# ChainUpZero/baby-plonk-rust

Hardware: AMD Instinct MI355X
Metric: g1_msm_scalar_muls_per_s (higher is better)
Workload: dtype u32 limbs (381-bit Fp Montgomery, 255-bit Fr)

## Files before the change

baby_plonk_rust_amd/csrc/capi_ctx.hip:

```cpp
#include <stdlib.h>
#include <string.h>

#include <algorithm>
#include <chrono>
#include <condition_variable>
#include <functional>
#include <mutex>
#include <thread>
#include <vector>

#include "ctx.hpp"

#include "capi_common.hpp"

using namespace bp;

namespace bp {

int fail(bp_ctx* ctx, int code, const char* what, hipError_t e, const char* file, int line) {
  if (ctx) {
    char buf[512];
    snprintf(buf, sizeof buf, "%s%s%s (%s:%d)", what, e != hipSuccess ? ": " : "", e != hipSuccess ? hipGetErrorString(e) : "", file,
             line);
    ctx->last_error = buf;
  }
  return code;
}

static thread_local bool tl_member_worker = false;

hipError_t stream_wait(hipStream_t st) {
  static const bool block = [] { const char* v = knob("BP_WAIT_BLOCK"); return v && *v == '1'; }();
  if (!block) {
    const auto limit = tl_member_worker ? std::chrono::microseconds(50) : std::chrono::microseconds(6000);
    const auto t0 = std::chrono::steady_clock::now();
    for (uint32_t spins = 0;; spins++) {
      const hipError_t e = hipStreamQuery(st);
      if (e != hipErrorNotReady) return e;
      __builtin_ia32_pause();
      if ((spins & 15) == 15 && std::chrono::steady_clock::now() - t0 > limit) break;
    }
  }
  return hipStreamSynchronize(st);
}

int ws_get(bp_ctx* ctx, const char* name, size_t bytes, void** out) {
  DevBuf& b = ctx->ws[name];
  if (bytes == 0) bytes = 16;
  if (b.cap < bytes) {
    if (b.p) {
      BP_HIP(ctx, stream_wait(ctx->stream));
      BP_HIP(ctx, hipFree(b.p));
      b.p = nullptr;
      b.cap = 0;
    }
    size_t cap = (bytes + 255) & ~(size_t)255;
    BP_HIP(ctx, hipMalloc(&b.p, cap));
    b.cap = cap;
  }
  *out = b.p;
  return BP_OK;
}

int ev_get(bp_ctx* ctx, const char* name, size_t count, unsigned flags, hipEvent_t** out) {
  std::vector<hipEvent_t>& ev = ctx->events[name];
  while (ev.size() < count) {
    hipEvent_t e;
    BP_HIP(ctx, hipEventCreateWithFlags(&e, flags));
    ev.push_back(e);
  }
  *out = ev.data();
  return BP_OK;
}

int pinned_get(bp_ctx* ctx, size_t bytes, void** out) {
  if (ctx->pinned_cap < bytes) {
    if (ctx->pinned) BP_HIP(ctx, hipHostFree(ctx->pinned));
    ctx->pinned = nullptr;
    ctx->pinned_cap = 0;
    size_t cap = std::max<size_t>(bytes, 64 * 1024);
    BP_HIP(ctx, hipHostMalloc(&ctx->pinned, cap, hipHostMallocDefault));
    ctx->pinned_cap = cap;
  }
  *out = ctx->pinned;
  return BP_OK;
}

}

int upload_fr(bp_ctx* ctx, const char* name, const void* host, size_t n, size_t cap_elems, int fmt, fr_t** out, uint32_t* d_bad) {
  fr_t* d;
  BP_TRY(ws_get(ctx, name, std::max(cap_elems, n) * sizeof(fr_t), (void**)&d));
  if (n) BP_HIP(ctx, hipMemcpyAsync(d, host, n * sizeof(fr_t), hipMemcpyHostToDevice, ctx->stream));
  if (fmt == BP_FR_BYTES_LE) BP_TRY(fr_convert_run(ctx, d, n, 0, d_bad));
  *out = d;
  return BP_OK;
}
int download_fr(bp_ctx* ctx, fr_t* d, void* host, size_t n, int fmt, const uint32_t* d_bad) {
  if (n == 0 && !d_bad) return BP_OK;
  uint32_t bad = 0;
  if (n && fmt == BP_FR_BYTES_LE) BP_TRY(fr_convert_run(ctx, d, n, 1));
  if (n) BP_HIP(ctx, hipMemcpyAsync(host, d, n * sizeof(fr_t), hipMemcpyDeviceToHost, ctx->stream));
  if (d_bad) BP_HIP(ctx, hipMemcpyAsync(&bad, d_bad, sizeof bad, hipMemcpyDeviceToHost, ctx->stream));
  BP_HIP(ctx, stream_wait(ctx->stream));
  if (bad) return BP_FAIL(ctx, BP_ERR_BAD_SCALAR, "vector element >= q");
  return BP_OK;
}

namespace bp {
struct MemberWorker {
  std::mutex mu;
  std::condition_variable cv;
  std::function<void()> job;
  bool has_job = false, done = true, stop = false;
  std::thread th;
  MemberWorker() : th([this] { loop(); }) {}
  ~MemberWorker() {
    {
      std::lock_guard<std::mutex> lk(mu);
      stop = true;
    }
    cv.notify_all();
    th.join();
  }
  void loop() {
    tl_member_worker = true;
    std::unique_lock<std::mutex> lk(mu);
    for (;;) {
      cv.wait(lk, [&] { return has_job || stop; });
      if (stop) return;
      std::function<void()> j = std::move(job);
      has_job = false;
      lk.unlock();
      j();
// ... 220 lines not shown
```

baby_plonk_rust_amd/csrc/ctx.hpp:

```cpp
#pragma once
#include <hip/hip_runtime.h>
#include <stdint.h>
#include <stdio.h>
#include <stdlib.h>
#include <map>
#include <string>
#include <vector>

#include "../../include/bp_msm_ntt.h"
#include "g1.hpp"
#include "g1_28.hpp"
#include "msm_plan.hpp"
#include "ntt_plan.hpp"
#include "prover_host.hpp"

namespace bp {

#ifdef BP_EXPERIMENT
inline const char* knob(const char* name) { return getenv(name); }
constexpr bool EXPERIMENT_BUILD = true;
#else
inline const char* knob(const char*) { return nullptr; }
constexpr bool EXPERIMENT_BUILD = false;
#endif
// ... 136 lines not shown
  const void* gen_table_ptr = nullptr;
  void* pinned = nullptr;
  size_t pinned_cap = 0;
};

namespace bp {

int fail(bp_ctx* ctx, int code, const char* what, hipError_t e, const char* file, int line);

inline int& device_guard_depth() {
  static thread_local int depth = 0;
  return depth;
}
struct DeviceGuard {
  int prev = -1;
  explicit DeviceGuard(int device) {
    if (device_guard_depth()++ == 0) (void)hipGetLastError();
    if (hipGetDevice(&prev) != hipSuccess) prev = -1;
    if (prev != device) (void)hipSetDevice(device);
  }
  ~DeviceGuard() {
    int cur = -1;
    if (prev >= 0 && hipGetDevice(&cur) == hipSuccess && cur != prev) (void)hipSetDevice(prev);
    device_guard_depth()--;
  }
  DeviceGuard(const DeviceGuard&) = delete;
  DeviceGuard& operator=(const DeviceGuard&) = delete;
};
inline bool is_group(const bp_ctx* ctx) { return ctx->members.size() > 1; }
inline int lift(bp_ctx* ctx, const bp_ctx* member, int rc) {
  if (rc != BP_OK && member != ctx) ctx->last_error = member->last_error;
  return rc;
}
inline bool peer_path(const bp_ctx* m, int other_device) {
  if (m->device != other_device) return true;
  if (m->leader && m->leader->rehearsal) return true;
  const char* v = knob("BP_FORCE_PEER_COPIES");
  return v && *v && *v != '0';
}

#define BP_HIP(ctx, call)                                                              \
  do {                                                                                 \
    hipError_t e__ = (call);                                                           \
    if (e__ != hipSuccess) return ::bp::fail(ctx, BP_ERR_HIP, #call, e__, __FILE__, __LINE__); \
  } while (0)
#define BP_FAIL(ctx, code, text) ::bp::fail(ctx, code, text, hipSuccess, __FILE__, __LINE__)
#define BP_TRY(expr)              \
  do {                            \
    int rc__ = (expr);            \
    if (rc__ != BP_OK) return rc__; \
  } while (0)

hipError_t stream_wait(hipStream_t st);
struct StreamDrain {
  hipStream_t st;
  ~StreamDrain() { (void)stream_wait(st); }
};

int ws_get(bp_ctx* ctx, const char* name, size_t bytes, void** out);
int ev_get(bp_ctx* ctx, const char* name, size_t count, unsigned flags, hipEvent_t** out);
int pinned_get(bp_ctx* ctx, size_t bytes, void** out);

struct MsmPending {
  bool empty = true, blob = false;
  bool tables = false;
  uint32_t c = 0, Wr = 0, n_planes = 0;
  uint32_t quads = 1;
  uint32_t J = 1;
  uint64_t adds = 0;
  const void* h_windows = nullptr;
};
int msm_launch(bp_ctx* ctx, const g1_affine28* d_points28, size_t n, const fr_t* d_scalars, int fmt, uint32_t table_c, size_t table_stride,
               int slot, void* d_blob, MsmPending* out);
int msm_launch_many(bp_ctx* ctx, const g1_affine28* d_points28, uint32_t J, const fr_t* const* d_scalars_each, const size_t* n_each, int fmt,
                    uint32_t table_c, size_t table_stride, int slot, void* d_blob, MsmPending* out);
int msm_blobs_combine(const uint8_t* blobs, size_t n_blobs, g1_proj* out);
int msm_blobs_sum_device_run(bp_ctx* ctx, const void* d_blobs, size_t n_blobs, void* d_out, bool wait = true);
int msm_blob_poisoned(const uint8_t* blobs, size_t n_blobs, uint32_t* rank);
int msm_blob_poison_run(bp_ctx* ctx, void* d_blob, int err, uint32_t rank);
int msm_finish(bp_ctx* ctx, const MsmPending& pend, g1_proj* host_out);
struct MsmFlight {
  bp_ctx* on = nullptr;
  MsmPending pend;
  bool launched = false;
  int rc = BP_OK;
  g1_proj out[MSM_MAX_BATCH];
};
inline int msm_flight_launched(MsmFlight& f, bp_ctx* on, int launch_rc) {
  f.on = on;
  f.rc = launch_rc;
  f.launched = launch_rc == BP_OK;
  return launch_rc;
}
int msm_finish_all(bp_ctx* ctx, MsmFlight* f, size_t count, int rc);
int msm_run(bp_ctx* ctx, const g1_affine28* d_points28, size_t n, const fr_t* d_scalars, int fmt, uint32_t table_c, size_t table_stride,
            g1_proj* host_out);
int msm_init_device(bp_ctx* ctx);
int commit_many(bp_ctx* ctx, uint64_t srs_handle, const fr_t* const* d_coeffs, const size_t* n, int k, g1_proj* out);
int srs_tables_run(bp_ctx* ctx, const g1_affine* d_points, const g1_affine28* d_points28, size_t n, uint32_t c, g1_affine28** d_table,
                   uint32_t* windows);
MsmKnobs msm_knobs();
int srs_to28_run(bp_ctx* ctx, const g1_affine* d_in, size_t n, g1_affine28** d_out);
int srs_to28_into(bp_ctx* ctx, const g1_affine* d_in, size_t n, g1_affine28* d_out);
int ntt_init_tables(bp_ctx* ctx);
int ntt_run(bp_ctx* ctx, fr_t* d_data, uint32_t log_n, int inverse, size_t batch, size_t stride);
NttKnobs ntt_knobs();
int ntt_tmp_buffer(bp_ctx* ctx, uint32_t log_n, fr_t** out);
int ntt_run_part(bp_ctx* ctx, const NttHostPlan& plan, fr_t* d_data, int inverse, size_t batch, size_t stride, int phase, uint32_t part, uint32_t parts);
int fr_convert_run(bp_ctx* ctx, fr_t* d, size_t n, int dir, uint32_t* d_bad = nullptr);
int fr_flag_noncanonical_run(bp_ctx* ctx, const fr_t* d, size_t n, uint32_t* d_bad, size_t row = 0, size_t stride = 0);
int fr_bad_word(bp_ctx* ctx, int fmt, uint32_t** d_bad);
int fr_binary_run(bp_ctx* ctx, const fr_t* a, size_t na, const fr_t* b, size_t nb, fr_t* out, size_t n, int op);
int fr_scalar_run(bp_ctx* ctx, const fr_t* a, const fr_t& s, fr_t* out, size_t n, int op);
int poly_eval_run(bp_ctx* ctx, const fr_t* d_coeffs, size_t n, const fr_t& x, fr_t* host_out, const uint32_t* d_bad = nullptr);
int poly_eval_many_run(bp_ctx* ctx, int k, const fr_t* const* d_coeffs, const size_t* n, const fr_t* x, fr_t* host_out);
int poly_div_run(bp_ctx* ctx, fr_t* d_a, size_t na, const fr_t* d_b, size_t nb, const fr_t& b0, const fr_t& b_lead, bool binomial,
                 fr_t* d_q, size_t nq);
int fr_nonzero_stats_run(bp_ctx* ctx, const fr_t* d_a, size_t n, size_t lo, size_t hi, size_t* eff_len, size_t* nonzero_in_range);
int fr_compact_nonzero_run(bp_ctx* ctx, fr_t* d_q, size_t* n);
int fr_squeeze_zeros_run(bp_ctx* ctx, fr_t* d_q, size_t* n);
int fr_scale_powers_run(bp_ctx* ctx, const fr_t* d_a, size_t n, const fr_t& w, fr_t* d_out);
int fr_synthetic_run(bp_ctx* ctx, fr_t* d_out, size_t n, uint64_t seed);
int fr_scan_mul_run(bp_ctx* ctx, const fr_t* d_in, size_t n, int reverse, int inclusive, fr_t* d_out, fr_t* d_total);
// ... 45 lines not shown
```

baby_plonk_rust_amd/csrc/g1_28.hpp:

```cpp
#pragma once
#include "fp28.hpp"
#include "g1.hpp"

namespace bp {

template <class To, uint64_t A, uint32_t VA>
BP_HD To widen28(const F28<A, VA>& a) {
  static_assert(A <= To::limb_bound && VA <= To::value_bound, "cannot narrow bounds");
  To r;
#pragma unroll
  for (int i = 0; i < N28; i++) r.l[i] = a.l[i];
  return r;
}

using C28 = F28<MASK28 + 8, 6>;
using PtY28 = F28<MASK28 + 8, 2>;

struct alignas(128) g1_affine28 {
  F28n x, y;
};
struct g1_proj28 {
  C28 x, y, z;
};
constexpr int PROJ28_WORDS = 44;
// ... 33 lines not shown
#pragma unroll
  for (int i = 0; i < N28; i++) zero.l[i] = 0;
  auto ny = norm28(sub28<2, 29>(zero, y));
  PtY28 a = widen28<PtY28>(ny), b = widen28<PtY28>(y), r;
#pragma unroll
  for (int i = 0; i < N28; i++) r.l[i] = neg ? a.l[i] : b.l[i];
  return r;
}

BP_HD void g1_add_mixed28(g1_proj28& acc, const F28n& x2, const PtY28& y2) {
  const C28 &X1 = acc.x, &Y1 = acc.y, &Z1 = acc.z;
  auto t0 = mul28(X1, x2);
  auto t1 = mul28(Y1, y2);
  auto t3 = mul28(add28(x2, y2), add28(X1, Y1));
  auto t3s = norm28(sub28<8, 30>(t3, add28(t0, t1)));
  auto t4 = add28(mul28(y2, Z1), Y1);
  auto y3a = norm28(add28(mul28(x2, Z1), X1));
  auto t0x3 = mulk28<3>(t0);
  auto t2 = norm28(mulk28<12>(Z1));
  auto z3 = add28(t1, t2);
  auto t1s = sub28<80, 29>(t1, t2);
  auto y3 = norm28(mulk28<12>(y3a));
  auto x3 = mul28_2(t3s, t1s, t4, neg28<128, 29>(y3));
  auto yo = mul28_2(t1s, z3, y3, t0x3);
  auto zo = mul28_2(z3, t4, t0x3, t3s);
  acc.x = widen28<C28>(x3);
  acc.y = widen28<C28>(yo);
  acc.z = widen28<C28>(zo);
}

BP_HD void g1_add28(g1_proj28& r, const g1_proj28& a, const g1_proj28& b) {
  auto t0 = mul28(a.x, b.x);
  auto t1 = mul28(a.y, b.y);
  auto t2 = mul28(a.z, b.z);
  auto t3 = norm28(sub28<8, 30>(mul28(add28(a.x, a.y), add28(b.x, b.y)), add28(t0, t1)));
  auto t4 = norm28(sub28<8, 30>(mul28(add28(a.y, a.z), add28(b.y, b.z)), add28(t1, t2)));
  auto y3a = norm28(sub28<8, 30>(mul28(add28(a.x, a.z), add28(b.x, b.z)), add28(t0, t2)));
  auto t0x3 = mulk28<3>(t0);
  auto t2b = norm28(mulk28<12>(t2));
  auto z3 = add28(t1, t2b);
  auto t1s = sub28<32, 29>(t1, t2b);
  auto y3 = norm28(mulk28<12>(y3a));
  auto x3 = mul28_2(t3, t1s, t4, neg28<128, 29>(y3));
  auto yo = mul28_2(t1s, z3, y3, t0x3);
  auto zo = mul28_2(z3, t4, t0x3, t3);
  r.x = widen28<C28>(x3);
  r.y = widen28<C28>(yo);
  r.z = widen28<C28>(zo);
}

using CoopProd = F28<MASK28, 2>;
using CoopSum = decltype(add28(C28(), C28()));

template <class U, class A, class B, class C>
BP_HD U select3_28(uint32_t which, const A& a, const B& b, const C& c) {
  const U ua = widen28<U>(a), ub = widen28<U>(b), uc = widen28<U>(c);
  U r;
#pragma unroll
  for (int i = 0; i < N28; i++) r.l[i] = which == 0 ? ua.l[i] : (which == 1 ? ub.l[i] : uc.l[i]);
  return r;
}
template <class A, class B, class C>
struct Union28 {
  static constexpr uint64_t lb = A::limb_bound > B::limb_bound ? (A::limb_bound > C::limb_bound ? A::limb_bound : C::limb_bound)
                                                               : (B::limb_bound > C::limb_bound ? B::limb_bound : C::limb_bound);
  static constexpr uint32_t vb = A::value_bound > B::value_bound ? (A::value_bound > C::value_bound ? A::value_bound : C::value_bound)
                                                                 : (B::value_bound > C::value_bound ? B::value_bound : C::value_bound);
  using type = F28<lb, vb>;
};

BP_HD CoopProd g1_add28_coop_a(uint32_t role, const g1_proj28& a, const g1_proj28& b) {
  const bool ux = role == 0 || role == 3 || role == 5, uy = role == 1 || role == 3 || role == 4, uz = role == 2 || role == 4 || role == 5;
  CoopSum u, v;
#pragma unroll
  for (int i = 0; i < N28; i++) {
    u.l[i] = (ux ? a.x.l[i] : 0u) + (uy ? a.y.l[i] : 0u) + (uz ? a.z.l[i] : 0u);
    v.l[i] = (ux ? b.x.l[i] : 0u) + (uy ? b.y.l[i] : 0u) + (uz ? b.z.l[i] : 0u);
  }
  return widen28<CoopProd>(mul28(u, v));
}
BP_HD C28 g1_add28_coop_b(uint32_t role, const CoopProd p[6]) {
  const CoopProd &t0 = p[0], &t1 = p[1], &t2 = p[2];
  auto t3 = norm28(sub28<8, 30>(p[3], add28(t0, t1)));
  auto t4 = norm28(sub28<8, 30>(p[4], add28(t1, t2)));
  auto y3a = norm28(sub28<8, 30>(p[5], add28(t0, t2)));
  auto t0x3 = norm28(mulk28<3>(t0));
  auto t2b = norm28(mulk28<12>(t2));
  auto z3 = norm28(add28(t1, t2b));
  auto t1s = norm28(sub28<32, 29>(t1, t2b));
  auto y3 = norm28(mulk28<12>(y3a));
  auto ny3 = norm28(neg28<128, 29>(y3));
  using P = typename Union28<decltype(t3), decltype(z3), decltype(t0x3)>::type;
  using Q = typename Union28<decltype(t1s), decltype(t1s), decltype(t3)>::type;
  using R = typename Union28<decltype(t4), decltype(t0x3), decltype(t4)>::type;
  using S = typename Union28<decltype(ny3), decltype(y3), decltype(z3)>::type;
  const uint32_t w = role < 3 ? role : 2;
  return widen28<C28>(mul28_2(select3_28<P>(w, t3, z3, t0x3), select3_28<Q>(w, t1s, t1s, t3), select3_28<R>(w, t4, t0x3, t4),
                              select3_28<S>(w, ny3, y3, z3)));
}

BP_HD void g1_double28(g1_proj28& r, const g1_proj28& p) {
  auto t0 = mul28(p.y, p.y);
  auto z8 = mulk28<8>(t0);
  auto t1 = mul28(p.y, p.z);
  auto t2 = norm28(mulk28<12>(mul28(p.z, p.z)));
  auto x3 = mul28(t2, z8);
  auto y3 = add28(t0, t2);
  auto zo = mul28(t1, z8);
  auto t0s = sub28<80, 30>(t0, mulk28<3>(t2));
  auto yo = add28(x3, mul28(t0s, y3));
  auto xo = mulk28<2>(mul28(t0s, mul28(p.x, p.y)));
  r.x = widen28<C28>(norm28(xo));
// ... 46 lines not shown
```

baby_plonk_rust_amd/csrc/msm.hip:

```cpp
#include <math.h>
#include <stdlib.h>
#include <string.h>

#include <vector>

#include "ctx.hpp"
#include "msm_kernels.hpp"

namespace bp {

static_assert(sizeof(proj28_slot) == MSM_SLOT_BYTES, "msm_plan.hpp sizes the workspaces by this");

MsmKnobs msm_knobs() { return msm_knobs_read(knob_u32); }

int srs_to28_run(bp_ctx* ctx, const g1_affine* d_in, size_t n, g1_affine28** d_out) {
  g1_affine28* d = nullptr;
  BP_HIP(ctx, hipMalloc((void**)&d, (n ? n : 1) * sizeof(g1_affine28)));
  if (n) hipLaunchKernelGGL(srs_to28, dim3((unsigned)((n + 255) / 256)), dim3(256), 0, ctx->stream, d_in, n, d);
  BP_HIP(ctx, hipGetLastError());
  *d_out = d;
  return BP_OK;
}

int srs_to28_into(bp_ctx* ctx, const g1_affine* d_in, size_t n, g1_affine28* d_out) {
// ... 92 lines not shown
  out->blob = d_blob != nullptr;
  const MsmHostPlan hp = msm_plan(J, n_each, table_c, table_stride, d_blob != nullptr, msm_knobs());
  if (hp.err == BP_ERR_INVALID_ARG) return BP_FAIL(ctx, hp.err, hp.what);
  out->J = J;
  if (hp.empty) {
    if (d_blob) {
      MsmBlobHeader hdr;
      memset(&hdr, 0, sizeof hdr);
      hdr.magic = MSM_BLOB_MAGIC;
      hipLaunchKernelGGL(msm_write_blob, dim3(1), dim3(64), 0, ctx->stream, (const proj28_slot*)nullptr, hdr, (uint8_t*)d_blob);
      BP_HIP(ctx, hipGetLastError());
    }
    return BP_OK;
  }
  if (slot < 0 || slot >= MSM_SLOTS) return BP_FAIL(ctx, BP_ERR_INVALID_ARG, "MSM result slot");
  if (hp.err) return BP_FAIL(ctx, hp.err, hp.what);
  const MsmPlan& plan = hp.dev;
  MsmScalars scalars_all;
  for (uint32_t j = 0; j < MSM_MAX_BATCH; j++) scalars_all.p[j] = j < J ? d_scalars_each[j] : nullptr;
  SortBufs b = {};
  uint32_t* long_list;
  proj28_slot *long_scratch, *bucket_sum, *partial, *roots = nullptr, *window_sum, *tmp[2] = {nullptr, nullptr};
  const struct { const char* name; size_t bytes; void** p; } buffers[] = {
      {"msm.ctl", hp.ws.ctl, (void**)&b.ctl},
      {"msm.counts", hp.ws.counts, (void**)&b.counts},
      {"msm.offsets", hp.ws.offsets, (void**)&b.offsets},
      {"msm.cursors", hp.ws.cursors, (void**)&b.cursors},
      {"msm.long_list", hp.ws.long_list, (void**)&long_list},
      {"msm.long_scratch", hp.ws.long_scratch, (void**)&long_scratch},
      {"msm.tile_sums", hp.ws.tile_sums, (void**)&b.tile_sums},
      {"msm.sorted", hp.ws.sorted, (void**)&b.sorted},
      {"msm.bucket_sum", hp.ws.bucket_sum, (void**)&bucket_sum},
      {"msm.partial", hp.ws.partial, (void**)&partial},
      {"msm.roots", hp.ws.roots, (void**)&roots},
      {"msm.window_sum", hp.ws.window_sum, (void**)&window_sum},
      {"msm.rkeys0", hp.ws.rkeys0, (void**)&b.keys[0]},
      {"msm.rvals0", hp.ws.rvals0, (void**)&b.vals[0]},
      {"msm.rkeys1", hp.ws.rkeys1, (void**)&b.keys[1]},
      {"msm.rvals1", hp.ws.rvals1, (void**)&b.vals[1]},
      {"msm.run_off", hp.ws.run_off, (void**)&b.run_off},
      {"msm.run_cnt", hp.ws.run_cnt, (void**)&b.run_cnt},
      {"msm.run_cur", hp.ws.run_cur, (void**)&b.run_cur},
      {"msm.run_long", hp.ws.run_long, (void**)&b.run_long},
      {"msm.planes_tmp0", hp.ws.planes_tmp0, (void**)&tmp[0]},
      {"msm.planes_tmp1", hp.ws.planes_tmp1, (void**)&tmp[1]},
  };
  for (const auto& w : buffers)
    if (w.bytes) BP_TRY(ws_get(ctx, w.name, w.bytes, w.p));
  constexpr size_t slot_bytes = (size_t)MSM_MAX_WINDOWS * sizeof(proj28_slot) + 16;
  uint8_t* h_base;
  BP_TRY(pinned_get(ctx, MSM_SLOTS * slot_bytes, (void**)&h_base));
  proj28_slot* h_windows = reinterpret_cast<proj28_slot*>(h_base + (size_t)slot * slot_bytes);
  const uint32_t total = plan.total, n_planes = hp.n_planes;
  uint32_t *offsets = b.offsets, *long_count = b.ctl, *status = b.ctl + 1, *long_ticket = b.ctl + 8 + PART_MAX;
  hipStream_t st = ctx->stream;
  BP_HIP(ctx, hipEventRecord(ctx->ev[0], st));
  BP_HIP(ctx, hipMemsetAsync(b.ctl, 0, (size_t)hp.ctl_zeroed * 4, st));
  if (hp.sort == 2) {
    level1_launch(st, hp, scalars_all, fmt, b, b.run_off, b.keys[0], b.vals[0]);
    (hp.packed ? final_runs_launch<true> : final_runs_launch<false>)(st, hp, b, b.keys[0], b.vals[0], b.run_off);
  } else {
    uint32_t* const run_off[2] = {b.run_off + 4,
                                  b.run_off + 8 + hp.n_final};
    level1_launch(st, hp, scalars_all, fmt, b, run_off[0], b.keys[1], b.vals[1]);
    uint32_t side = 1;
    if (hp.lv[1]) {
      const dim3 grid(hp.gx2, 1u << hp.lv[0]);
      BP_HIP(ctx, hipMemsetAsync(b.run_cnt, 0, (size_t)hp.n_sub * 4, st));
      hipLaunchKernelGGL(msm_radix_count, grid, dim3(1024), 0, st, b.keys[side], run_off[0], hp.shift2, hp.lv[1], b.run_cnt);
      hipLaunchKernelGGL(scan_tile_sums, dim3(hp.scan_tiles), dim3(256), 0, st, b.run_cnt, hp.n_sub, b.tile_sums);
      hipLaunchKernelGGL(scan_block_sums, dim3(1), dim3(256), 0, st, b.tile_sums, hp.scan_tiles, run_off[1] + hp.n_sub);
      hipLaunchKernelGGL(scan_apply, dim3(hp.scan_tiles), dim3(256), 0, st, b.run_cnt, hp.n_sub, b.tile_sums, run_off[1], b.run_cur);
      hipLaunchKernelGGL(msm_radix_scatter, grid, dim3(1024), RADIX_SLICE * 9, st, b.keys[side], b.vals[side], run_off[0], hp.shift2, hp.lv[1], b.run_cur,
                         b.keys[side ^ 1], b.vals[side ^ 1]);
      side ^= 1;
    }
    final_runs_launch<false>(st, hp, b, b.keys[side], b.vals[side], run_off[hp.lv[1] ? 1 : 0]);
  }
  BP_HIP(ctx, hipEventRecord(ctx->ev[1], st));
  hipLaunchKernelGGL(msm_accumulate<2>, dim3(hp.acc_grid), dim3(256), 0, st, d_points28, b.sorted, offsets, plan, bucket_sum, partial);
  BP_HIP(ctx, hipEventRecord(ctx->ev[2], st));
  if (hp.by_edges)
    hipLaunchKernelGGL(msm_fixup_edges, dim3(hp.fixup_grid), dim3(256), 0, st, offsets, plan, bucket_sum, partial, long_count, long_list, hp.long_cap);
  else if (table_c)
    hipLaunchKernelGGL(msm_fixup<2>, dim3(hp.fixup_grid), dim3(256), 0, st, offsets, plan, bucket_sum, partial, long_count, long_list, hp.long_cap);
  else
    hipLaunchKernelGGL(msm_fixup<1>, dim3(hp.fixup_grid), dim3(256), 0, st, offsets, plan, bucket_sum, partial, long_count, long_list, hp.long_cap);
  hipLaunchKernelGGL(msm_fixup_long, dim3(512), dim3(256), 256 * sizeof(proj28_slot), st, offsets, plan, bucket_sum, partial, long_count, long_list, hp.long_cap,
                     long_scratch, long_ticket);
  uint32_t* const status_out = reinterpret_cast<uint32_t*>(window_sum + n_planes);
  const proj28_slot* in = bucket_sum;
  for (uint32_t i = 0; i < hp.n_steps; i++) {
    const MsmTreeStep& s = hp.step[i];
    const bool last = s.out == MSM_OUT_FINAL;
    proj28_slot* out_nodes = last ? (table_c ? window_sum : roots) : tmp[s.out];
    const dim3 grid(s.gx, s.gy);
    if (s.kind == MSM_STEP_LEVEL01) {
      hipLaunchKernelGGL(msm_planes_level01, grid, dim3(256), 0, st, offsets, in, s.nodes, out_nodes);
    } else if (s.kind == MSM_STEP_LEVEL) {
      hipLaunchKernelGGL(msm_planes_level, grid, dim3(256), 0, st, offsets, in, s.k, s.nodes, out_nodes);
    } else {
      uint32_t* so = last && table_c ? status_out : (uint32_t*)nullptr;
      if (s.k == 0) hipLaunchKernelGGL(msm_planes_step<true>, grid, dim3(256), s.lds, st, offsets, in, s.k, s.m, out_nodes, status, offsets + total, so);
      else hipLaunchKernelGGL(msm_planes_step<false>, grid, dim3(256), s.lds, st, offsets, in, s.k, s.m, out_nodes, status, offsets + total, so);
    }
    in = out_nodes;
  }
  if (!table_c)
    hipLaunchKernelGGL(msm_planes_window_quads, dim3(plan.W), dim3(64), 0, st, roots, plan.c, hp.quads, window_sum, status, offsets + total, status_out);
  BP_HIP(ctx, hipGetLastError());
  if (d_blob) {
    MsmBlobHeader hdr;
    memset(&hdr, 0, sizeof hdr);
    hdr.magic = MSM_BLOB_MAGIC;
    hdr.c = plan.c;
    hdr.Wr = table_c ? 1 : hp.Wr;
    hdr.n_planes = n_planes;
    hdr.tables = table_c != 0;
    hdr.quads = table_c ? 0u : hp.quads;
    hipLaunchKernelGGL(msm_write_blob, dim3(1), dim3(256), 0, st, window_sum, hdr, (uint8_t*)d_blob);
    BP_HIP(ctx, hipGetLastError());
  } else {
    BP_HIP(ctx, hipMemcpyAsync(h_windows, window_sum, (size_t)n_planes * sizeof(proj28_slot) + 8, hipMemcpyDeviceToHost, st));
  }
  BP_HIP(ctx, hipEventRecord(ctx->ev[3], st));
  out->empty = false;
  out->tables = table_c != 0;
  out->c = plan.c;
  out->Wr = table_c ? 1 : hp.Wr;
  out->n_planes = n_planes;
  out->quads = hp.quads;
  out->adds = hp.entries;
  out->h_windows = h_windows;
  msm_plan_path(hp, ctx->msm_path);
  return BP_OK;
}

static void host_quad_horner(g1_proj& out, const g1_proj* quads, uint32_t W, uint32_t c, uint32_t nq) {
  g1_proj acc = g1_identity();
  uint32_t prev = 0;
  bool first = true;
  for (uint32_t w = W; w-- > 0;)
    for (uint32_t j = nq; j-- > 0;) {
      const uint32_t pos = c * w + 4 * j;
      if (first) {
        acc = quads[(size_t)w * nq + j];
        first = false;
      } else {
        for (uint32_t d = pos; d < prev; d++) g1_double(acc, acc);
        g1_add(acc, acc, quads[(size_t)w * nq + j]);
      }
      prev = pos;
    }
  out = acc;
}

static void host_plane_horner(g1_proj& out, const g1_proj* planes, uint32_t W, uint32_t c) {
  g1_proj acc = g1_identity();
  for (uint32_t w = W; w-- > 0;) {
    const g1_proj* p = planes + (size_t)w * c;
    for (uint32_t j = c; j-- > 0;) {
      g1_double(acc, acc);
      if (j + 1 < c) g1_add(acc, acc, p[1 + j]);
    }
    g1_add(acc, acc, p[0]);
  }
  out = acc;
}

int msm_finish(bp_ctx* ctx, const MsmPending& pend, g1_proj* host_out) {
  ctx->msm_async_pending = false;
  if (pend.empty) {
    for (uint32_t j = 0; host_out && j < pend.J; j++) host_out[j] = g1_identity();
    ctx->msm_accumulate_ms = ctx->msm_total_ms = 0;
    ctx->msm_adds = 0;
    if (pend.blob) BP_HIP(ctx, stream_wait(ctx->stream));
    return BP_OK;
  }
  BP_HIP(ctx, stream_wait(ctx->stream));
  BP_HIP(ctx, hipEventElapsedTime(&ctx->msm_accumulate_ms, ctx->ev[1], ctx->ev[2]));
  BP_HIP(ctx, hipEventElapsedTime(&ctx->msm_total_ms, ctx->ev[0], ctx->ev[3]));
  ctx->msm_c = pend.c;
  ctx->msm_tables = pend.tables;
  ctx->msm_adds = pend.adds;
  if (pend.blob) {
    if (host_out) *host_out = g1_identity();
    return BP_OK;
  }
  const proj28_slot* h_windows = static_cast<const proj28_slot*>(pend.h_windows);
  const uint32_t n_planes = pend.n_planes;
  const uint32_t* tail = reinterpret_cast<const uint32_t*>(h_windows + n_planes);
  if (tail[0]) return BP_FAIL(ctx, BP_ERR_BAD_SCALAR, "scalar >= q in a canonical-bytes input");
  ctx->msm_adds = tail[1];
  std::vector<g1_proj> windows(n_planes);
  for (uint32_t w = 0; w < n_planes; w++) windows[w] = slot_to_proj(&h_windows[w]);
  if (pend.tables) {
    for (uint32_t j = 0; j < pend.J; j++)
      host_plane_horner(host_out[j], windows.data() + (size_t)j * pend.c, pend.Wr, pend.c);
  } else {
    host_quad_horner(*host_out, windows.data(), pend.Wr, pend.c, pend.quads);
  }
  return BP_OK;
}

int msm_blobs_combine(const uint8_t* blobs, size_t n_blobs, g1_proj* out) {
  g1_proj total = g1_identity();
  std::vector<bool> done(n_blobs, false);
  for (size_t i = 0; i < n_blobs; i++) {
    MsmBlobHeader h;
    memcpy(&h, blobs + i * BP_MSM_BLOB_BYTES, sizeof h);
    if (h.magic != MSM_BLOB_MAGIC || h.n_planes > (uint32_t)MSM_MAX_WINDOWS) return BP_ERR_INVALID_ARG;
    if (h.err != 0) return h.err < 0 && h.err >= BP_ERR_COMM ? h.err : BP_ERR_INVALID_ARG;
    if (h.tables > 1) return BP_ERR_INVALID_ARG;
    if (h.n_planes != 0) {
      const bool width_ok = h.c >= 2 && h.c <= (uint32_t)MSM_MAX_TABLE_C;
      const uint32_t per = h.tables ? h.c : (h.quads ? h.quads : 1u);
      if (!width_ok || h.Wr < 1 || per > 8 * 4 || h.n_planes != h.Wr * per) return BP_ERR_INVALID_ARG;
    }
    if (h.status) return BP_ERR_BAD_SCALAR;
  }
  for (size_t i = 0; i < n_blobs; i++) {
    if (done[i]) continue;
    MsmBlobHeader h;
    memcpy(&h, blobs + i * BP_MSM_BLOB_BYTES, sizeof h);
    done[i] = true;
    if (h.n_planes == 0) continue;
    std::vector<g1_proj> sum(h.n_planes);
    const proj28_slot* slots = reinterpret_cast<const proj28_slot*>(blobs + i * BP_MSM_BLOB_BYTES + sizeof(MsmBlobHeader));
    for (uint32_t w = 0; w < h.n_planes; w++) sum[w] = slot_to_proj(&slots[w]);
    for (size_t k = i + 1; k < n_blobs; k++) {
      MsmBlobHeader g;
      memcpy(&g, blobs + k * BP_MSM_BLOB_BYTES, sizeof g);
      if (done[k] || g.c != h.c || g.Wr != h.Wr || g.n_planes != h.n_planes || g.tables != h.tables || g.quads != h.quads) continue;
      done[k] = true;
      const proj28_slot* sk = reinterpret_cast<const proj28_slot*>(blobs + k * BP_MSM_BLOB_BYTES + sizeof(MsmBlobHeader));
      for (uint32_t w = 0; w < h.n_planes; w++) g1_add(sum[w], sum[w], slot_to_proj(&sk[w]));
    }
    g1_proj part;
    if (h.tables) host_plane_horner(part, sum.data(), h.Wr, h.c);
    else host_quad_horner(part, sum.data(), h.Wr, h.c, h.quads ? h.quads : 1u);
    g1_add(total, total, part);
  }
  *out = total;
  return BP_OK;
}

int msm_blob_poisoned(const uint8_t* blobs, size_t n_blobs, uint32_t* rank) {
  for (size_t i = 0; i < n_blobs; i++) {
    MsmBlobHeader h;
    memcpy(&h, blobs + i * BP_MSM_BLOB_BYTES, sizeof h);
    if (h.magic == MSM_BLOB_MAGIC && h.err != 0) {
      if (rank) *rank = h.err_rank;
      return h.err < 0 && h.err >= BP_ERR_COMM ? h.err : BP_ERR_INVALID_ARG;
    }
  }
// ... 31 lines not shown
```

baby_plonk_rust_amd/csrc/msm_kernels.hpp:

```cpp
#pragma once
#include "g1.hpp"
#include "g1_28.hpp"
#include "msm_digits.hpp"
#include "msm_plan.hpp"

namespace bp {

struct MsmScalars { const fr_t* p[MSM_MAX_BATCH]; };

__device__ __forceinline__ uint32_t digit_bucket(int32_t d) { return (uint32_t)(d < 0 ? -d : d) - 1u; }

extern __shared__ uint32_t msm_lds_hist[];

constexpr uint32_t SCAN_PER_LANE = 16;

__device__ __forceinline__ uint32_t block_exclusive_scan_256(uint32_t v, uint32_t* lds, uint32_t& block_total) {
  const uint32_t lane = threadIdx.x & 63, wave = threadIdx.x >> 6;
  uint32_t incl = v;
#pragma unroll
  for (int d = 1; d < 64; d <<= 1) {
    uint32_t n = __shfl_up(incl, d, 64);
    if (lane >= (uint32_t)d) incl += n;
  }
  if (lane == 63) lds[wave] = incl;
// ... 468 lines not shown

__device__ __forceinline__ g1_affine load_affine(const g1_affine* __restrict__ p) {
  g1_affine r;
  const uint4* q = reinterpret_cast<const uint4*>(p);
  uint4 v[6];
#pragma unroll
  for (int j = 0; j < 6; j++) v[j] = q[j];
#pragma unroll
  for (int j = 0; j < 3; j++) {
    r.x.l[4 * j] = v[j].x; r.x.l[4 * j + 1] = v[j].y; r.x.l[4 * j + 2] = v[j].z; r.x.l[4 * j + 3] = v[j].w;
    r.y.l[4 * j] = v[j + 3].x; r.y.l[4 * j + 1] = v[j + 3].y; r.y.l[4 * j + 2] = v[j + 3].z; r.y.l[4 * j + 3] = v[j + 3].w;
  }
  return r;
}
__device__ __forceinline__ g1_affine28 load_affine28(const g1_affine28* __restrict__ p) {
  g1_affine28 r;
  const uint4* q = reinterpret_cast<const uint4*>(p);
  uint4 v[7];
#pragma unroll
  for (int j = 0; j < 7; j++) v[j] = q[j];
  uint32_t w[28];
#pragma unroll
  for (int j = 0; j < 7; j++) { w[4 * j] = v[j].x; w[4 * j + 1] = v[j].y; w[4 * j + 2] = v[j].z; w[4 * j + 3] = v[j].w; }
#pragma unroll
  for (int j = 0; j < N28; j++) { r.x.l[j] = w[j]; r.y.l[j] = w[N28 + j]; }
  return r;
}
struct proj28_slot { uint4 q[11]; };
__device__ __forceinline__ void store_proj28(proj28_slot* __restrict__ dst, const g1_proj28& p) {
  uint32_t w[PROJ28_WORDS];
#pragma unroll
  for (int j = 0; j < N28; j++) { w[j] = p.x.l[j]; w[N28 + j] = p.y.l[j]; w[2 * N28 + j] = p.z.l[j]; }
  w[42] = 0; w[43] = 0;
#pragma unroll
  for (int j = 0; j < 11; j++) dst->q[j] = make_uint4(w[4 * j], w[4 * j + 1], w[4 * j + 2], w[4 * j + 3]);
}
__device__ __forceinline__ g1_proj28 load_proj28(const proj28_slot* __restrict__ src) {
  uint32_t w[PROJ28_WORDS];
#pragma unroll
  for (int j = 0; j < 11; j++) { uint4 v = src->q[j]; w[4 * j] = v.x; w[4 * j + 1] = v.y; w[4 * j + 2] = v.z; w[4 * j + 3] = v.w; }
  g1_proj28 p;
#pragma unroll
  for (int j = 0; j < N28; j++) { p.x.l[j] = w[j]; p.y.l[j] = w[N28 + j]; p.z.l[j] = w[2 * N28 + j]; }
  return p;
}
__device__ __forceinline__ bool is_blank28(const g1_proj28& p) {
  uint32_t z = 0;
#pragma unroll
  for (int j = 0; j < N28; j++) z |= p.z.l[j];
  return z == 0;
}

constexpr uint32_t COOP = 8;
__device__ __forceinline__ g1_proj28 g1_add28_coop(const g1_proj28& a, const g1_proj28& b) {
  const uint32_t role = threadIdx.x & (COOP - 1);
  const CoopProd mine = g1_add28_coop_a(role, a, b);
  CoopProd p[6];
#pragma unroll
  for (int r = 0; r < 6; r++) {
#pragma unroll
    for (int j = 0; j < N28; j++) p[r].l[j] = (uint32_t)__shfl((int)mine.l[j], r, COOP);
  }
  const C28 coord = g1_add28_coop_b(role, p);
  g1_proj28 out;
#pragma unroll
  for (int j = 0; j < N28; j++) {
    out.x.l[j] = (uint32_t)__shfl((int)coord.l[j], 0, COOP);
    out.y.l[j] = (uint32_t)__shfl((int)coord.l[j], 1, COOP);
    out.z.l[j] = (uint32_t)__shfl((int)coord.l[j], 2, COOP);
  }
  return out;
}

__global__ void __launch_bounds__(256) srs_to28(const g1_affine* __restrict__ in, size_t n, g1_affine28* __restrict__ out) {
  size_t i = (size_t)blockIdx.x * blockDim.x + threadIdx.x;
  if (i >= n) return;
  g1_affine28 r = g1_affine_to_28(load_affine(&in[i]));
  uint4* q = reinterpret_cast<uint4*>(&out[i]);
  uint32_t w[28];
#pragma unroll
  for (int j = 0; j < N28; j++) { w[j] = r.x.l[j]; w[N28 + j] = r.y.l[j]; }
#pragma unroll
  for (int j = 0; j < 7; j++) q[j] = make_uint4(w[4 * j], w[4 * j + 1], w[4 * j + 2], w[4 * j + 3]);
}

constexpr int TABLE_GROUP = 16;
__device__ __forceinline__ M28 one_m28() {
  M28 r;
#pragma unroll
  for (int j = 0; j < N28; j++) r.l[j] = One28::limb(j);
  return r;
}
template <bool RADIX>
__global__ void __launch_bounds__(256) srs_window_tables(const g1_affine28* __restrict__ in28, size_t n, uint32_t c, uint32_t W, uint32_t radix,
                                                         g1_affine28* __restrict__ table) {
  size_t i = (size_t)blockIdx.x * blockDim.x + threadIdx.x;
  if (i >= n) return;
  const g1_affine28 a = load_affine28(&in28[i]);
  uint32_t nz = 0;
#pragma unroll
  for (int j = 0; j < N28; j++) nz |= a.x.l[j] | a.y.l[j];
  const bool inf = nz == 0;
  g1_proj28 p = g1_identity28();
  if (!inf) {
    p.x = widen28<C28>(a.x);
    p.y = widen28<C28>(a.y);
    p.z = widen28<C28>(one_m28());
  }
  g1_proj28 row[TABLE_GROUP];
  M28 prefix[TABLE_GROUP];
  const M28 one = one_m28();
  for (uint32_t w0 = 1; w0 < W; w0 += TABLE_GROUP) {
    const uint32_t cnt = W - w0 < (uint32_t)TABLE_GROUP ? W - w0 : (uint32_t)TABLE_GROUP;
    for (uint32_t j = 0; j < cnt; j++) {
      if (RADIX) g1_mul_small28(p, p, radix, 32 - __clz(radix));
      else
// ... 248 lines not shown
    }
    g1_proj28 tot = block_tree_sum28(acc, per < blockDim.x ? per : blockDim.x);
    if (!split) {
      if (threadIdx.x == 0) store_proj28(&bucket_sum[g], tot);
      __syncthreads();
      continue;
    }
    if (threadIdx.x == 0) {
      store_proj28(&scratch[(size_t)k * FIXUP_LONG_SLICES + y], tot);
      __builtin_amdgcn_fence(__ATOMIC_RELEASE, "agent");
      asm volatile("s_waitcnt vmcnt(0)" ::: "memory");
      const uint32_t t = atomicAdd(&ticket[k], 1u);
      if (t == FIXUP_LONG_SLICES - 1) {
        ticket[k] = 0;
        __builtin_amdgcn_fence(__ATOMIC_ACQUIRE, "agent");
        asm volatile("s_waitcnt vmcnt(0)" ::: "memory");
      }
      arrived = t;
    }
    __syncthreads();
    if (arrived == FIXUP_LONG_SLICES - 1) {
      g1_proj28 v = g1_identity28();
      if (threadIdx.x < FIXUP_LONG_SLICES) v = load_proj28(&scratch[(size_t)k * FIXUP_LONG_SLICES + threadIdx.x]);
      g1_proj28 sum = block_tree_sum28(v, FIXUP_LONG_SLICES);
      if (threadIdx.x == 0) store_proj28(&bucket_sum[g], sum);
    }
    __syncthreads();
  }
}

__device__ __forceinline__ g1_proj28 block_tree_sum28(g1_proj28 v, uint32_t live) {
  proj28_slot* tree = reinterpret_cast<proj28_slot*>(msm_lds_tree);
  store_proj28(&tree[threadIdx.x], v);
  __syncthreads();
  uint32_t stride = 1;
  while (stride < live) stride <<= 1;
  const uint32_t group = threadIdx.x / COOP, n_groups = blockDim.x / COOP;
  for (stride >>= 1; stride > 0; stride >>= 1) {
    for (uint32_t i = group; i < stride; i += n_groups) {
      if (i + stride < live) {
        g1_proj28 a = load_proj28(&tree[i]), b = load_proj28(&tree[i + stride]);
        a = g1_add28_coop(a, b);
        if ((threadIdx.x & (COOP - 1)) == 0) store_proj28(&tree[i], a);
      }
    }
    __syncthreads();
  }
  return load_proj28(&tree[0]);
}


__device__ __forceinline__ proj28_slot* planes_tree(proj28_slot* cur, proj28_slot* nxt, uint32_t levels, bool planes) {
  const uint32_t group = threadIdx.x / COOP, n_groups = blockDim.x / COOP;
  const bool lead = (threadIdx.x & (COOP - 1)) == 0;
  for (uint32_t k = 0; k < levels; k++) {
    const uint32_t merges = 1u << (levels - k - 1);
    const uint32_t in_per = planes ? k + 1 : 1, out_per = planes ? k + 2 : 1, adds = merges * in_per;
    for (uint32_t item = group; item < adds; item += n_groups) {
      const uint32_t m = item / in_per, v = item - m * in_per;
      const proj28_slot* L = cur + (size_t)(2 * m) * in_per;
      g1_proj28 a = load_proj28(&L[v]), b = load_proj28(&L[in_per + v]);
      if (!(is_blank28(a) && is_blank28(b))) a = g1_add28_coop(a, b);
      if (lead) store_proj28(&nxt[(size_t)m * out_per + v], a);
    }
    if (planes)
      for (uint32_t m = threadIdx.x; m < merges; m += blockDim.x) nxt[(size_t)m * out_per + k + 1] = cur[(size_t)(2 * m + 1) * in_per];
    __syncthreads();
    proj28_slot* t = cur; cur = nxt; nxt = t;
  }
  return cur;
}

__global__ void __launch_bounds__(256, 2)
msm_planes_level(const uint32_t* __restrict__ offsets, const proj28_slot* __restrict__ in, uint32_t k, uint32_t n_out,
                 proj28_slot* __restrict__ out) {
  const uint64_t item = (uint64_t)blockIdx.x * blockDim.x + threadIdx.x;
  const uint32_t per = k + 1, node = (uint32_t)(item / per), v = (uint32_t)(item - (uint64_t)node * per);
  if (node >= n_out) return;
  const proj28_slot* L = in + (size_t)(2 * (size_t)node) * per;
  g1_proj28 a = load_proj28(&L[v]), b = load_proj28(&L[per + v]);
  proj28_slot* o = out + (size_t)node * (per + 1);
  if (v == 0) store_proj28(&o[per], b);
  if (!(is_blank28(a) && is_blank28(b))) g1_add28(a, a, b);
  store_proj28(&o[v], a);
}

__global__ void __launch_bounds__(256, 2)
msm_planes_level01(const uint32_t* __restrict__ offsets, const proj28_slot* __restrict__ in, uint32_t n_out, proj28_slot* __restrict__ out) {
  const uint32_t node = blockIdx.x * blockDim.x + threadIdx.x;
  if (node >= n_out) return;
  const size_t g = 4 * (size_t)node;
  const uint32_t o0 = offsets[g], o1 = offsets[g + 1], o2 = offsets[g + 2], o3 = offsets[g + 3], o4 = offsets[g + 4];
  proj28_slot* o = out + (size_t)node * 3;
  if (o4 == o0) {
    const g1_proj28 blank = g1_identity28();
    store_proj28(&o[0], blank);
    store_proj28(&o[1], blank);
    store_proj28(&o[2], blank);
    return;
  }
  {
    g1_proj28 s1 = o2 != o1 ? load_proj28(&in[g + 1]) : g1_identity28();
    {
      g1_proj28 a01 = o1 != o0 ? load_proj28(&in[g]) : g1_identity28();
      g1_add28(a01, a01, s1);
      store_proj28(&o[0], a01);
    }
    const g1_proj28 s3 = o4 != o3 ? load_proj28(&in[g + 3]) : g1_identity28();
    g1_add28(s1, s1, s3);
    store_proj28(&o[1], s1);
  }
  g1_proj28 a23 = o3 != o2 ? load_proj28(&in[g + 2]) : g1_identity28();
  {
    const g1_proj28 s3 = o4 != o3 ? load_proj28(&in[g + 3]) : g1_identity28();
    g1_add28(a23, a23, s3);
  }
  store_proj28(&o[2], a23);
  asm volatile("s_waitcnt vmcnt(0)" ::: "memory");
  g1_proj28 a01 = load_proj28(&o[0]);
  g1_add28(a01, a01, a23);
  store_proj28(&o[0], a01);
}

template <bool LEAF>
__global__ void __launch_bounds__(256, 2)
msm_planes_step(const uint32_t* __restrict__ offsets, const proj28_slot* __restrict__ in, uint32_t k, uint32_t m,
                proj28_slot* __restrict__ out, const uint32_t* __restrict__ status_in, const uint32_t* __restrict__ entries_in,
                uint32_t* __restrict__ status_out) {
  proj28_slot* buf = reinterpret_cast<proj28_slot*>(msm_lds_tree);
  const uint32_t w = blockIdx.x, v = blockIdx.y, nin = 1u << m, c = k + m + 1;
  if (status_out && v == 0 && w == 0 && threadIdx.x == 0) { status_out[0] = *status_in; status_out[1] = *entries_in; }
  if (threadIdx.x < nin) {
    const size_t node = ((size_t)w << m) + threadIdx.x;
    if (LEAF) {
      if (offsets[node + 1] != offsets[node]) buf[threadIdx.x] = in[node];
      else store_proj28(&buf[threadIdx.x], g1_identity28());
    } else {
      buf[threadIdx.x] = in[node * (k + 1) + v];
    }
  }
  __syncthreads();
  const proj28_slot* root = planes_tree(buf, buf + nin, m, v == 0);
  if (v == 0) {
    if (threadIdx.x == 0) out[(size_t)w * c] = root[0];
    else if (threadIdx.x <= m) out[(size_t)w * c + k + threadIdx.x] = root[threadIdx.x];
  } else if (threadIdx.x == 0) {
    out[(size_t)w * c + v] = root[0];
  }
}

__global__ void __launch_bounds__(64) msm_planes_window_quads(const proj28_slot* __restrict__ roots, uint32_t c, uint32_t nq, proj28_slot* __restrict__ window_sum,
                                                              const uint32_t* __restrict__ status_in, const uint32_t* __restrict__ entries_in,
                                                              uint32_t* __restrict__ status_out) {
  __shared__ proj28_slot part[4];
  const uint32_t w = blockIdx.x, grp = threadIdx.x / COOP, j = grp >> 1, h = grp & 1;
  const bool lead = (threadIdx.x & (COOP - 1)) == 0;
  if (w == 0 && threadIdx.x == 0) { status_out[0] = *status_in; status_out[1] = *entries_in; }
  const proj28_slot* r = roots + (size_t)w * c;
  const uint32_t np = c - 1, p0 = 4 * j + 2 * h, p1 = p0 + 1;
  auto pick = [](bool c, const g1_proj28& a, const g1_proj28& b) {
    g1_proj28 o;
#pragma unroll
    for (int i = 0; i < N28; i++) {
      o.x.l[i] = c ? a.x.l[i] : b.x.l[i];
      o.y.l[i] = c ? a.y.l[i] : b.y.l[i];
      o.z.l[i] = c ? a.z.l[i] : b.z.l[i];
    }
    return o;
  };
  const g1_proj28 blank = g1_identity28();
  const bool have1 = j < nq && p1 < np, have0 = j < nq && p0 < np;
  g1_proj28 t = pick(have1, load_proj28(&r[have1 ? 1 + p1 : 0]), blank);
  t = g1_add28_coop(t, t);
  t = g1_add28_coop(t, pick(have0, load_proj28(&r[have0 ? 1 + p0 : 0]), blank));
  t = g1_add28_coop(t, pick(h != 0, t, pick(j == 0, load_proj28(&r[0]), blank)));
  t = g1_add28_coop(t, pick(h != 0, t, blank));
  if (h && lead && j < 4) store_proj28(&part[j], t);
  __syncthreads();
  if (h) return;
  t = g1_add28_coop(t, load_proj28(&part[j]));
  if (lead && j < nq) store_proj28(&window_sum[(size_t)w * nq + j], t);
}

}
```

Baseline: 400.4 million.

## Write MSM window sums directly to mapped host memory and signal via flag

When the last tree step is a plain step kernel on the table path, its outputs go straight into coherent, mapped pinned host memory. A last-block ticket then sets a host-visible flag, so the host can start the Horner epilogue while the stream is still draining, with no D2H memcpy. The planes tree now lets three cooperating lanes each store one output coordinate instead of only the lead lane storing all of it, and select3 uses bitmask picks instead of branches. The risks are slower device writes into host-coherent memory, the pinned buffer now being mapped and coherent, and the ordering correctness of the fence and ticket.

```diff
diff --git a/baby_plonk_rust_amd/csrc/capi_ctx.hip b/baby_plonk_rust_amd/csrc/capi_ctx.hip
--- a/baby_plonk_rust_amd/csrc/capi_ctx.hip
+++ b/baby_plonk_rust_amd/csrc/capi_ctx.hip
@@ -44,6 +44,18 @@
   return hipStreamSynchronize(st);
 }
 
+bool flag_wait(const volatile uint32_t* flag) {
+  static const bool block = [] { const char* v = knob("BP_WAIT_BLOCK"); return v && *v == '1'; }();
+  if (block) return false;
+  const auto limit = tl_member_worker ? std::chrono::microseconds(50) : std::chrono::microseconds(6000);
+  const auto t0 = std::chrono::steady_clock::now();
+  for (uint32_t spins = 0;; spins++) {
+    if (__atomic_load_n(flag, __ATOMIC_ACQUIRE)) return true;
+    __builtin_ia32_pause();
+    if ((spins & 63) == 63 && std::chrono::steady_clock::now() - t0 > limit) return false;
+  }
+}
+
 int ws_get(bp_ctx* ctx, const char* name, size_t bytes, void** out) {
   DevBuf& b = ctx->ws[name];
   if (bytes == 0) bytes = 16;
@@ -79,7 +91,7 @@
     ctx->pinned = nullptr;
     ctx->pinned_cap = 0;
     size_t cap = std::max<size_t>(bytes, 64 * 1024);
-    BP_HIP(ctx, hipHostMalloc(&ctx->pinned, cap, hipHostMallocDefault));
+    BP_HIP(ctx, hipHostMalloc(&ctx->pinned, cap, hipHostMallocMapped | hipHostMallocCoherent));
     ctx->pinned_cap = cap;
   }
   *out = ctx->pinned;
diff --git a/baby_plonk_rust_amd/csrc/ctx.hpp b/baby_plonk_rust_amd/csrc/ctx.hpp
--- a/baby_plonk_rust_amd/csrc/ctx.hpp
+++ b/baby_plonk_rust_amd/csrc/ctx.hpp
@@ -212,6 +212,7 @@
   } while (0)
 
 hipError_t stream_wait(hipStream_t st);
+bool flag_wait(const volatile uint32_t* flag);
 struct StreamDrain {
   hipStream_t st;
   ~StreamDrain() { (void)stream_wait(st); }
@@ -229,6 +230,7 @@
   uint32_t J = 1;
   uint64_t adds = 0;
   const void* h_windows = nullptr;
+  const uint32_t* h_flag = nullptr;
 };
 int msm_launch(bp_ctx* ctx, const g1_affine28* d_points28, size_t n, const fr_t* d_scalars, int fmt, uint32_t table_c, size_t table_stride,
                int slot, void* d_blob, MsmPending* out);
diff --git a/baby_plonk_rust_amd/csrc/g1_28.hpp b/baby_plonk_rust_amd/csrc/g1_28.hpp
--- a/baby_plonk_rust_amd/csrc/g1_28.hpp
+++ b/baby_plonk_rust_amd/csrc/g1_28.hpp
@@ -109,12 +109,14 @@
 using CoopProd = F28<MASK28, 2>;
 using CoopSum = decltype(add28(C28(), C28()));
 
+BP_HD uint32_t pick28(uint32_t mask, uint32_t a, uint32_t b) { return (a & mask) | (b & ~mask); }
 template <class U, class A, class B, class C>
 BP_HD U select3_28(uint32_t which, const A& a, const B& b, const C& c) {
   const U ua = widen28<U>(a), ub = widen28<U>(b), uc = widen28<U>(c);
+  const uint32_t m0 = 0u - (uint32_t)(which == 0), m1 = 0u - (uint32_t)(which == 1);
   U r;
 #pragma unroll
-  for (int i = 0; i < N28; i++) r.l[i] = which == 0 ? ua.l[i] : (which == 1 ? ub.l[i] : uc.l[i]);
+  for (int i = 0; i < N28; i++) r.l[i] = pick28(m0, ua.l[i], pick28(m1, ub.l[i], uc.l[i]));
   return r;
 }
 template <class A, class B, class C>
diff --git a/baby_plonk_rust_amd/csrc/msm.hip b/baby_plonk_rust_amd/csrc/msm.hip
--- a/baby_plonk_rust_amd/csrc/msm.hip
+++ b/baby_plonk_rust_amd/csrc/msm.hip
@@ -168,6 +168,13 @@
   BP_TRY(pinned_get(ctx, MSM_SLOTS * slot_bytes, (void**)&h_base));
   proj28_slot* h_windows = reinterpret_cast<proj28_slot*>(h_base + (size_t)slot * slot_bytes);
   const uint32_t total = plan.total, n_planes = hp.n_planes;
+  const bool direct = table_c && !d_blob && hp.n_steps && hp.step[hp.n_steps - 1].kind == MSM_STEP_STEP;
+  proj28_slot* d_slot = nullptr;
+  volatile uint32_t* h_flag = reinterpret_cast<uint32_t*>(h_windows + n_planes) + 2;
+  if (direct) {
+    BP_HIP(ctx, hipHostGetDevicePointer((void**)&d_slot, h_windows, 0));
+    *h_flag = 0;
+  }
   uint32_t *offsets = b.offsets, *long_count = b.ctl, *status = b.ctl + 1, *long_ticket = b.ctl + 8 + PART_MAX;
   hipStream_t st = ctx->stream;
   BP_HIP(ctx, hipEventRecord(ctx->ev[0], st));
@@ -209,16 +216,18 @@
   for (uint32_t i = 0; i < hp.n_steps; i++) {
     const MsmTreeStep& s = hp.step[i];
     const bool last = s.out == MSM_OUT_FINAL;
-    proj28_slot* out_nodes = last ? (table_c ? window_sum : roots) : tmp[s.out];
+    proj28_slot* out_nodes = last ? (table_c ? (direct ? d_slot : window_sum) : roots) : tmp[s.out];
     const dim3 grid(s.gx, s.gy);
     if (s.kind == MSM_STEP_LEVEL01) {
       hipLaunchKernelGGL(msm_planes_level01, grid, dim3(256), 0, st, offsets, in, s.nodes, out_nodes);
     } else if (s.kind == MSM_STEP_LEVEL) {
       hipLaunchKernelGGL(msm_planes_level, grid, dim3(256), 0, st, offsets, in, s.k, s.nodes, out_nodes);
     } else {
-      uint32_t* so = last && table_c ? status_out : (uint32_t*)nullptr;
-      if (s.k == 0) hipLaunchKernelGGL(msm_planes_step<true>, grid, dim3(256), s.lds, st, offsets, in, s.k, s.m, out_nodes, status, offsets + total, so);
-      else hipLaunchKernelGGL(msm_planes_step<false>, grid, dim3(256), s.lds, st, offsets, in, s.k, s.m, out_nodes, status, offsets + total, so);
+      const bool hand_over = last && direct;
+      uint32_t* so = last && table_c ? (hand_over ? reinterpret_cast<uint32_t*>(d_slot + n_planes) : status_out) : (uint32_t*)nullptr;
+      uint32_t *ticket = hand_over ? b.ctl + 3 : (uint32_t*)nullptr, *flag = hand_over ? so + 2 : (uint32_t*)nullptr;
+      if (s.k == 0) hipLaunchKernelGGL(msm_planes_step<true>, grid, dim3(256), s.lds, st, offsets, in, s.k, s.m, out_nodes, status, offsets + total, so, ticket, flag);
+      else hipLaunchKernelGGL(msm_planes_step<false>, grid, dim3(256), s.lds, st, offsets, in, s.k, s.m, out_nodes, status, offsets + total, so, ticket, flag);
     }
     in = out_nodes;
   }
@@ -236,7 +245,7 @@
     hdr.quads = table_c ? 0u : hp.quads;
     hipLaunchKernelGGL(msm_write_blob, dim3(1), dim3(256), 0, st, window_sum, hdr, (uint8_t*)d_blob);
     BP_HIP(ctx, hipGetLastError());
-  } else {
+  } else if (!direct) {
     BP_HIP(ctx, hipMemcpyAsync(h_windows, window_sum, (size_t)n_planes * sizeof(proj28_slot) + 8, hipMemcpyDeviceToHost, st));
   }
   BP_HIP(ctx, hipEventRecord(ctx->ev[3], st));
@@ -248,6 +257,7 @@
   out->quads = hp.quads;
   out->adds = hp.entries;
   out->h_windows = h_windows;
+  out->h_flag = direct ? const_cast<const uint32_t*>(h_flag) : nullptr;
   msm_plan_path(hp, ctx->msm_path);
   return BP_OK;
 }
@@ -293,6 +303,23 @@
     if (pend.blob) BP_HIP(ctx, stream_wait(ctx->stream));
     return BP_OK;
   }
+  const proj28_slot* h_windows = static_cast<const proj28_slot*>(pend.h_windows);
+  const uint32_t n_planes = pend.n_planes;
+  const uint32_t* tail = reinterpret_cast<const uint32_t*>(h_windows + n_planes);
+  auto epilogue = [&]() -> int {
+    if (tail[0]) return BP_FAIL(ctx, BP_ERR_BAD_SCALAR, "scalar >= q in a canonical-bytes input");
+    std::vector<g1_proj> windows(n_planes);
+    for (uint32_t w = 0; w < n_planes; w++) windows[w] = slot_to_proj(&h_windows[w]);
+    if (pend.tables) {
+      for (uint32_t j = 0; j < pend.J; j++)
+        host_plane_horner(host_out[j], windows.data() + (size_t)j * pend.c, pend.Wr, pend.c);
+    } else {
+      host_quad_horner(*host_out, windows.data(), pend.Wr, pend.c, pend.quads);
+    }
+    return BP_OK;
+  };
+  const bool early = pend.h_flag && flag_wait(pend.h_flag);
+  int rc = early ? epilogue() : BP_OK;
   BP_HIP(ctx, stream_wait(ctx->stream));
   BP_HIP(ctx, hipEventElapsedTime(&ctx->msm_accumulate_ms, ctx->ev[1], ctx->ev[2]));
   BP_HIP(ctx, hipEventElapsedTime(&ctx->msm_total_ms, ctx->ev[0], ctx->ev[3]));
@@ -303,20 +330,9 @@
     if (host_out) *host_out = g1_identity();
     return BP_OK;
   }
-  const proj28_slot* h_windows = static_cast<const proj28_slot*>(pend.h_windows);
-  const uint32_t n_planes = pend.n_planes;
-  const uint32_t* tail = reinterpret_cast<const uint32_t*>(h_windows + n_planes);
-  if (tail[0]) return BP_FAIL(ctx, BP_ERR_BAD_SCALAR, "scalar >= q in a canonical-bytes input");
-  ctx->msm_adds = tail[1];
-  std::vector<g1_proj> windows(n_planes);
-  for (uint32_t w = 0; w < n_planes; w++) windows[w] = slot_to_proj(&h_windows[w]);
-  if (pend.tables) {
-    for (uint32_t j = 0; j < pend.J; j++)
-      host_plane_horner(host_out[j], windows.data() + (size_t)j * pend.c, pend.Wr, pend.c);
-  } else {
-    host_quad_horner(*host_out, windows.data(), pend.Wr, pend.c, pend.quads);
-  }
-  return BP_OK;
+  if (!early) rc = epilogue();
+  if (rc == BP_OK) ctx->msm_adds = tail[1];
+  return rc;
 }
 
 int msm_blobs_combine(const uint8_t* blobs, size_t n_blobs, g1_proj* out) {
diff --git a/baby_plonk_rust_amd/csrc/msm_kernels.hpp b/baby_plonk_rust_amd/csrc/msm_kernels.hpp
--- a/baby_plonk_rust_amd/csrc/msm_kernels.hpp
+++ b/baby_plonk_rust_amd/csrc/msm_kernels.hpp
@@ -544,7 +544,7 @@
 }
 
 constexpr uint32_t COOP = 8;
-__device__ __forceinline__ g1_proj28 g1_add28_coop(const g1_proj28& a, const g1_proj28& b) {
+__device__ __forceinline__ C28 g1_add28_coop_coord(const g1_proj28& a, const g1_proj28& b) {
   const uint32_t role = threadIdx.x & (COOP - 1);
   const CoopProd mine = g1_add28_coop_a(role, a, b);
   CoopProd p[6];
@@ -553,7 +553,10 @@
 #pragma unroll
     for (int j = 0; j < N28; j++) p[r].l[j] = (uint32_t)__shfl((int)mine.l[j], r, COOP);
   }
-  const C28 coord = g1_add28_coop_b(role, p);
+  return g1_add28_coop_b(role, p);
+}
+__device__ __forceinline__ g1_proj28 g1_add28_coop(const g1_proj28& a, const g1_proj28& b) {
+  const C28 coord = g1_add28_coop_coord(a, b);
   g1_proj28 out;
 #pragma unroll
   for (int j = 0; j < N28; j++) {
@@ -908,16 +911,26 @@
 
 __device__ __forceinline__ proj28_slot* planes_tree(proj28_slot* cur, proj28_slot* nxt, uint32_t levels, bool planes) {
   const uint32_t group = threadIdx.x / COOP, n_groups = blockDim.x / COOP;
-  const bool lead = (threadIdx.x & (COOP - 1)) == 0;
+  const uint32_t role = threadIdx.x & (COOP - 1);
   for (uint32_t k = 0; k < levels; k++) {
     const uint32_t merges = 1u << (levels - k - 1);
     const uint32_t in_per = planes ? k + 1 : 1, out_per = planes ? k + 2 : 1, adds = merges * in_per;
     for (uint32_t item = group; item < adds; item += n_groups) {
       const uint32_t m = item / in_per, v = item - m * in_per;
       const proj28_slot* L = cur + (size_t)(2 * m) * in_per;
-      g1_proj28 a = load_proj28(&L[v]), b = load_proj28(&L[in_per + v]);
-      if (!(is_blank28(a) && is_blank28(b))) a = g1_add28_coop(a, b);
-      if (lead) store_proj28(&nxt[(size_t)m * out_per + v], a);
+      const g1_proj28 a = load_proj28(&L[v]), b = load_proj28(&L[in_per + v]);
+      proj28_slot* dst = &nxt[(size_t)m * out_per + v];
+      if (!(is_blank28(a) && is_blank28(b))) {
+        const C28 coord = g1_add28_coop_coord(a, b);
+        if (role < 3) {
+          uint2* d2 = reinterpret_cast<uint2*>(dst) + 7 * role;
+#pragma unroll
+          for (int j = 0; j < N28 / 2; j++) d2[j] = make_uint2(coord.l[2 * j], coord.l[2 * j + 1]);
+          if (role == 2) d2[7] = make_uint2(0u, 0u);
+        }
+      } else if (role == 0) {
+        store_proj28(dst, a);
+      }
     }
     if (planes)
       for (uint32_t m = threadIdx.x; m < merges; m += blockDim.x) nxt[(size_t)m * out_per + k + 1] = cur[(size_t)(2 * m + 1) * in_per];
@@ -982,7 +995,7 @@
 __global__ void __launch_bounds__(256, 2)
 msm_planes_step(const uint32_t* __restrict__ offsets, const proj28_slot* __restrict__ in, uint32_t k, uint32_t m,
                 proj28_slot* __restrict__ out, const uint32_t* __restrict__ status_in, const uint32_t* __restrict__ entries_in,
-                uint32_t* __restrict__ status_out) {
+                uint32_t* __restrict__ status_out, uint32_t* __restrict__ done_ticket, uint32_t* __restrict__ host_flag) {
   proj28_slot* buf = reinterpret_cast<proj28_slot*>(msm_lds_tree);
   const uint32_t w = blockIdx.x, v = blockIdx.y, nin = 1u << m, c = k + m + 1;
   if (status_out && v == 0 && w == 0 && threadIdx.x == 0) { status_out[0] = *status_in; status_out[1] = *entries_in; }
@@ -1002,6 +1015,15 @@
     else if (threadIdx.x <= m) out[(size_t)w * c + k + threadIdx.x] = root[threadIdx.x];
   } else if (threadIdx.x == 0) {
     out[(size_t)w * c + v] = root[0];
+  }
+  if (host_flag) {
+    __threadfence_system();
+    __syncthreads();
+    if (threadIdx.x == 0 && atomicAdd(done_ticket, 1u) == gridDim.x * gridDim.y - 1) {
+      __threadfence_system();
+      *done_ticket = 0;
+      __hip_atomic_store(host_flag, 1u, __ATOMIC_RELEASE, __HIP_MEMORY_SCOPE_SYSTEM);
+    }
   }
 }
 
```

Result: no change. 403.6 million, median of 6 (+0.8%).
